# martingoe/physics

Hardware: AMD Instinct MI355X
Metric: rigid_body_steps_per_sec (higher is better)
Workload: dtype f32; 1 GPU; C5_256000_tower; n_bodies=256000, bodies_per_gpu=256000, dt_nanos=16666667, preroll_steps=30, rccl_ranks=0

## Files before the change

physics_amd/csrc/abi.hip:

```cpp
#include <algorithm>
#include <atomic>
#include <cmath>
#include <cstdlib>
#include <cstring>
#include <limits>
#include <string>
#include <vector>

#include "kernels.hpp"

namespace phys {
static thread_local std::string g_error;
void set_error(const std::string& msg) { g_error = msg; }
const char* get_error() { return g_error.c_str(); }
}

using namespace phys;

namespace phys {
void poll_snapshots(phys_world* w);
StepCounters* snapshot_acquire(phys_world* w) {
    const uint32_t k = w->snap_next;
    if (w->snap_pending[k]) {
        (void)hipEventSynchronize(w->snap_event[k]);
// ... 32 lines not shown
        hint.full_rounds = c.color_rounds;
    } else if (exact) {
        hint.color_rounds = c.color_rounds;
    } else {
        hint.recent_new[hint.recent_pos % 8] = c.n_new_manifolds;
        hint.recent_rounds[hint.recent_pos++ % 8] = c.color_rounds;
        uint32_t mx = 0, mn = 0;
        for (int q = 0; q < 8; ++q) {
            mx = hint.recent_rounds[q] > mx ? hint.recent_rounds[q] : mx;
            mn = hint.recent_new[q] > mn ? hint.recent_new[q] : mn;
        }
        hint.color_rounds = mx;
        hint.n_new = mn;
    }
    for (int q = 0; q < kMaxColors; ++q) hint.color_count[q] = c.color_count[q];
}

void poll_snapshots(phys_world* w) {
    for (int i = 0; i < phys_world::kSnapRing; ++i) {
        const uint32_t k = (w->snap_next + i) % phys_world::kSnapRing;
        if (!w->snap_pending[k]) continue;
        if (hipEventQuery(w->snap_event[k]) != hipSuccess) {
            (void)hipGetLastError();
            continue;
        }
        const StepCounters& c = *w->h_snap[k];
        w->snap_pending[k] = false;
        w->host_sticky_overflow |= c.overflow | c.sticky_overflow;
        if (c.n_static_pairs > w->static_pairs_seen) w->static_pairs_seen = c.n_static_pairs;
        if (c.overflow) continue;
        hint_adopt(w->hint, c, w->snap_full[k], false);
    }
}
}

namespace phys {
static std::atomic<int> g_worlds[64];
int worlds_on_device(int device) { return g_worlds[device & 63].load(std::memory_order_relaxed); }
bool gpu_is_exclusive(const phys_world* w) {
    return (w->cfg.flags & PHYS_FLAG_EXCLUSIVE_GPU) && !(w->cfg.flags & PHYS_FLAG_SHARED_GPU) && worlds_on_device(w->device) == 1;
}

static PlanInputs plan_inputs(const phys_world* w) {
    PlanInputs in;
    in.flags = w->cfg.flags; in.solver_iterations = w->cfg.solver_iterations;
    in.n = w->n; in.n_owned = w->n_owned; in.max_manifolds = w->max_manifolds;
    in.grid_table_size = w->grid_table_size;
    in.cus = w->cus;
    in.exclusive = gpu_is_exclusive(w);
    in.warm = w->warm;
    in.flow_vel = w->flow_vel.p != nullptr;
    in.cluster_count = w->cluster_count; in.cluster_dynamic = w->cluster_dynamic;
    in.ctab_valid = w->ctab_valid; in.color_epoch = w->color_epoch;
    uint64_t st_cap = 0;
    const uint32_t* st_pairs = nullptr;
    const float* st_geo = nullptr;
    static_narrow_args(w, &st_cap, &st_pairs, &st_geo);
    const uint64_t n_ground = (w->cfg.flags & PHYS_FLAG_GROUND_PLANE) ? (uint32_t)w->n : 0u;
    in.statics = st_pairs != nullptr;
    in.capsules = w->body_capsules || (in.statics && w->static_capsules) || w->max_ghosts > 0;
    in.filters = w->body_filters_set || (in.statics && w->static_filters_set) || (n_ground && w->ground_filter_set) || w->max_ghosts > 0;
    in.materials = materials_active(w);
    in.np_items = n_ground + w->max_pairs + st_cap;
    return in;
}

template <class Parse>
static auto debug_env(const char* name, Parse parse) -> std::optional<decltype(parse(""))> {
    if (const char* v = getenv(name)) return parse(v);
    return std::nullopt;
}
static bool debug_set(const char* name) { return getenv(name) != nullptr; }
static uint64_t parse_u64(const char* v) { return strtoull(v, nullptr, 10); }
static bool parse_one(const char* v) { return v[0] == '1'; }

const DebugSwitches& debug_switches() {
    static const DebugSwitches d = [] {
        DebugSwitches s;
        s.no_cluster = debug_set("PHYS_DEBUG_NO_CLUSTER");
        s.cluster_min = debug_env("PHYS_DEBUG_CLUSTER_MIN", parse_u64);
        s.clusters_per_cu = debug_env("PHYS_DEBUG_CLUSTERS_PER_CU", atoi);
        s.cluster_dynamic = debug_set("PHYS_DEBUG_CLUSTER_DYNAMIC");
        s.cluster_cap = debug_env("PHYS_DEBUG_CLUSTER_CAP", parse_u64).value_or(0);
        s.flow_max = debug_env("PHYS_DEBUG_FLOW_MAX", parse_u64);
        s.flow_quad_max = debug_env("PHYS_DEBUG_FLOW_QUAD_MAX", parse_u64).value_or(0);
        s.flow_pipeline = debug_env("PHYS_DEBUG_FLOW_PIPELINE", parse_one);
        s.np_early_probe = debug_env("PHYS_DEBUG_NP_EARLY_PROBE", parse_one);
        s.no_flow_preference = debug_set("PHYS_DEBUG_NO_FLOW_PREFERENCE");
        s.flow_stall = debug_set("PHYS_DEBUG_FLOW_STALL");
        s.flow_epoch = debug_env("PHYS_DEBUG_FLOW_EPOCH", [](const char* v) { return (uint32_t)strtoul(v, nullptr, 0); }).value_or(0u);
        s.ctab_slots = debug_env("PHYS_DEBUG_CTAB_SLOTS", parse_u64).value_or(0);
        s.color_kernel_lane = debug_env("PHYS_DEBUG_COLOR_KERNEL", [](const char* v) { return v[0] == 'l'; });
        s.np_threads = debug_env("PHYS_DEBUG_NP_THREADS", atoi).value_or(0);
        s.pair_lanes = debug_env("PHYS_DEBUG_PAIR_LANES", atoi).value_or(0);
        s.pair_kernel_brick = debug_env("PHYS_DEBUG_PAIR_KERNEL", [](const char* v) { return v[0] != 'b' || v[1] == 'r'; });
        s.brick_stage = debug_env("PHYS_DEBUG_BRICK_STAGE", atoi).value_or(0);
        s.raycast_stats = debug_set("PHYS_DEBUG_RAYCAST_STATS");
        return s;
    }();
    return d;
}
}

static float duration_as_secs_f32(uint64_t nanos_total) {
    const uint64_t secs = nanos_total / 1000000000ull;
    const uint32_t nanos = (uint32_t)(nanos_total % 1000000000ull);
    return (float)secs + (float)nanos / 1.0e9f;
}

phys_world::~phys_world() {
    (void)hipSetDevice(device);
    if (stream) (void)hipStreamSynchronize(stream);
    prof.destroy();
    for (int k = 0; k < kSnapRing; ++k) {
        if (h_snap[k]) (void)hipHostFree(h_snap[k]);
        if (snap_event[k]) (void)hipEventDestroy(snap_event[k]);
    }
    if (h_counters) (void)hipHostFree(h_counters);
    if (stream) (void)hipStreamDestroy(stream);
}

template <typename T>
static int32_t upload_pairs(phys_world* w, DevBuf<T>& dst, const std::vector<T>& h, bool& set_flag) {
    if (!h.empty()) PHYS_HIP_TRY(hipMemcpyAsync(dst.p, h.data(), sizeof(T) * h.size(), hipMemcpyHostToDevice, w->stream));
    PHYS_HIP_TRY(hipStreamSynchronize(w->stream));
    set_flag = true;
    return PHYS_OK;
}
template <typename T>
static int32_t download_body_pairs(phys_world* w, const DevBuf<T>& src, std::vector<T>& h) {
    h.resize(2 * w->n_owned);
    if (!h.empty()) PHYS_HIP_TRY(hipMemcpyAsync(h.data(), src.p, sizeof(T) * h.size(), hipMemcpyDeviceToHost, w->stream));
    PHYS_HIP_TRY(hipStreamSynchronize(w->stream));
    return PHYS_OK;
}

struct Staging : StageLayout {
    phys_world* w;
    DevBuf<uint8_t>& buf;
    Staging(phys_world* w, DevBuf<uint8_t>& buf) : w(w), buf(buf) {}
    int32_t reserve() {
        if (refused) return fail(PHYS_ERR_INVALID_ARG, "more arrays than a staging buffer holds");
        PHYS_HIP_TRY(buf.resize(total));
        return PHYS_OK;
    }
    template <typename T>
    T* at(Slot<T> s) const { return StageLayout::at(buf.p, s); }
    int32_t copy(hipMemcpyKind kind) {
        for (int k = 0; k < count; ++k) {
            const Array& a = arrays[k];
            if (kind == hipMemcpyHostToDevice) PHYS_HIP_TRY(hipMemcpyAsync(buf.p + a.offset, a.host, a.bytes, kind, w->stream));
            else PHYS_HIP_TRY(hipMemcpyAsync(a.host, buf.p + a.offset, a.bytes, kind, w->stream));
        }
        return PHYS_OK;
    }
};

template <class Batch, class... Kind>
static int32_t query_device(phys_world* w, const Batch& b, Kind... kind) {
    ENTER(w);
    if (const char* bad = args_error(kind..., b)) return fail(PHYS_ERR_INVALID_ARG, bad);
    if (b.n == 0) return PHYS_OK;
    return launch_query(w, kind..., b);
}

template <class Batch, class... Kind>
// ... 1073 lines not shown
```

physics_amd/csrc/cluster.hip:

```cpp
#include <algorithm>
#include <cstdio>
#include <cstdlib>
#include <mutex>
#include <vector>

#include "handoff.hpp"

namespace phys {


static size_t seg_count_offset(uint64_t n) { return ((size_t)2 * n + 3) & ~(size_t)3; }

int32_t cluster_assign(phys_world* w, const float* pos ) {
    w->cluster_count = 0;
    w->seg_count_dirty = false;
    w->seg_count_bins = 0;
    const uint64_t n = w->n, n_owned = w->n_owned;
    const DebugSwitches& dbg = debug_switches();
    w->cluster_dynamic = false;
    w->cluster_homes_valid = false;
    if (dbg.no_cluster || n_owned < kClusterMinBodies || !w->flow_vel.p) return PHYS_OK;
    const int per_cu_max = cluster_per_cu_max(w->all_diag_inertia);
    const ClusterFit fit = cluster_fit(n_owned, cluster_per_cu_first(per_cu_max, dbg), w->cus, 0u);
    if (dbg.cluster_dynamic || !fit.ok) {
// ... 106 lines not shown
                if (seen == 0xFFFFFFFFu || seen == key) break;
                s = (s + 1u) & (uint32_t)(kKeysSlots - 1);
            }
            my_slot[j] = s;
            my_rank[j] = atomicAdd(&t_cnt[s], 1u);
            if (hb != kNoHome && hb != owner) atomicOr(&body_shared[2 * (size_t)b + (c >> 5)], 1u << (c & 31u));
        }
        __syncthreads();
        for (uint32_t s = threadIdx.x; s < (uint32_t)kKeysSlots; s += 256u)
            if (t_cnt[s]) t_base[s] = atomicAdd(&seg_count[t_key[s]], t_cnt[s]);
        __syncthreads();
#pragma unroll
        for (int j = 0; j < kKeysItems; ++j) {
            const uint64_t m = base + (uint64_t)j * 256u + threadIdx.x;
            if (m < M) man_rank[m] = my_slot[j] == 0xFFFFFFFFu ? 0xFFFFFFFFu : t_base[my_slot[j]] + my_rank[j];
        }
        __syncthreads();
    }
    __syncthreads();
    if (threadIdx.x < PHYS_MAX_COLORS) {
        const uint32_t cnt = s_hist[threadIdx.x];
        if (cnt) atomicAdd(&ctr->color_count[threadIdx.x], cnt);
        const unsigned long long live = __ballot(cnt != 0u);
        if (threadIdx.x == 0 && live) atomicMax(&ctr->n_colors, 64u - (uint32_t)__clzll((long long)live));
    }
}

__global__ __launch_bounds__(256) void k_cluster_place(uint64_t max_manifolds, const uint32_t* __restrict__ man_a,
                                                       const uint32_t* __restrict__ man_b, const uint32_t* __restrict__ man_color,
                                                       const uint32_t* __restrict__ cluster_slot, uint32_t slots, uint32_t clusters,
                                                       const uint32_t* __restrict__ seg_start, const uint32_t* __restrict__ man_rank,
                                                       uint32_t* __restrict__ row_src, const StepCounters* __restrict__ ctr,
                                                       StepCounters* snap_out ) {
    counters_snapshot(ctr, snap_out);
    const uint32_t raw = ctr->n_manifolds;
    const uint32_t M = (uint64_t)raw < max_manifolds ? raw : (uint32_t)max_manifolds;
    for (uint32_t m = blockIdx.x * blockDim.x + threadIdx.x; m < M; m += gridDim.x * blockDim.x) {
        const uint32_t r = man_rank[m];
        if (r == 0xFFFFFFFFu) continue;
        const uint32_t a = man_a[m], b = man_b[m];
        const uint32_t ha = cluster_home(cluster_slot, a, slots);
        const uint32_t hb = (ha != kNoHome || PHYS_IS_STATIC_PARTNER(b)) ? kNoHome : cluster_home(cluster_slot, b, slots);
        row_src[seg_start[cluster_row_owner(a, ha, hb, clusters) * PHYS_MAX_COLORS + man_color[m]] + r] = m;
    }
}


void launch_cluster_sort(phys_world* w, const ColorPlan& plan, StepCounters* snap_out) {
    hipStream_t s = w->stream;
    const uint32_t bins = w->cluster_count * PHYS_MAX_COLORS;
    PHYS_PROF(w, PHYS_STAGE_ROWS);
    if (w->cluster_dynamic && w->cluster_homes_valid) ++w->cluster_age;
    if (w->cluster_dynamic && !w->cluster_homes_valid) {
        w->cluster_homes_valid = true;
        w->cluster_age = 0;
        const uint32_t n = (uint32_t)w->n, homes = w->cluster_count * w->cluster_slots;
        const dim3 g((n + 255) / 256), b(256);
        (void)hipMemsetAsync(w->active_flag.p, 0, ((size_t)n + 4) * 4, s);
        (void)hipMemsetAsync(w->cluster_body.p, 0xFF, (size_t)homes * 4, s);
        hipLaunchKernelGGL(k_active_flags, g, b, 0, s, (uint32_t)w->n_owned, w->color_state.p, w->bucket_of.p, w->bucket_cursor.p,
                           w->bucket_start.p, w->active_flag.p);
        const uint32_t n4 = (n + 3u) & ~3u;
        launch_exclusive_scan(w, w->active_flag.p, n4, w->active_rank.p, false, w->scan_block_sums.p);
        hipLaunchKernelGGL(k_cluster_homes, g, b, 0, s, n, (uint32_t)w->n_owned, w->color_state.p, w->bucket_of.p, w->bucket_cursor.p,
                           w->bucket_start.p, w->active_rank.p, n4, homes, w->cluster_slot.p, w->cluster_body.p, w->counters.p);
    }
    const bool self_zeroing = scan_is_one_launch(bins) && !w->seg_count_dirty;
    w->seg_count_dirty = !scan_is_one_launch(bins);
    uint32_t* seg_count = w->body_shared.p + seg_count_offset(w->n);
    (void)hipMemsetAsync(w->body_shared.p, 0, self_zeroing ? (size_t)w->n * 8 : (seg_count_offset(w->n) + (size_t)std::max<uint32_t>(bins, w->seg_count_bins)) * 4, s);
    w->seg_count_bins = bins;
    hipLaunchKernelGGL(k_cluster_keys, dim3(plan.cluster_key_blocks), dim3(256), 0, s, w->max_manifolds, w->man_a.p, w->man_b.p, w->man_color.p,
                       w->cluster_slot.p, w->cluster_slots, w->cluster_count, seg_count, w->man_rank.p, w->body_shared.p, w->counters.p);
    launch_exclusive_scan(w, seg_count, bins, w->seg_start.p, scan_is_one_launch(bins), w->scan_block_sums.p);
    hipLaunchKernelGGL(k_cluster_place, dim3(plan.cluster_sort_blocks), dim3(256), 0, s, w->max_manifolds, w->man_a.p, w->man_b.p, w->man_color.p,
                       w->cluster_slot.p, w->cluster_slots, w->cluster_count, w->seg_start.p, w->man_rank.p, w->row_src.p, w->counters.p, snap_out);
}

struct ClusterRowArrays { float4* all; uint64_t cap; };

__device__ __forceinline__ void cluster_loads_landed() { __builtin_amdgcn_s_waitcnt(0x0F70); }

constexpr int kClusterThreads = 256;
template <bool DIAG, bool GUARDED, bool MAT>
__global__ __launch_bounds__(kClusterThreads, DIAG ? kClusterPerCuDiag : kClusterPerCuFull) void k_solve_cluster(StepCounters* ctr, uint32_t iterations, uint32_t epoch,
                                                                  ClusterRowArrays rows, float friction,
                                                                  const float* __restrict__ inv_inertia, uint32_t inertia_stride,
                                                                  float* vel, const float* __restrict__ pos, float* flow_vel, uint32_t n_bodies,
                                                                  const uint32_t* __restrict__ cluster_body,
                                                                  const uint32_t* __restrict__ body_shared,
                                                                  const uint32_t* __restrict__ seg_start, uint32_t slots,
                                                                  long long timeout_ticks, uint32_t attempt,
                                                                  uint32_t last_attempt, long long arrive_ticks,
                                                                  uint32_t warm_sweep , const uint32_t* __restrict__ row_src,
                                                                  float* __restrict__ man_imp ) {
    extern __shared__ __attribute__((aligned(16))) float4 s_lds[];
    float4* s_body = s_lds;
    uint32_t* s_seg = reinterpret_cast<uint32_t*>(s_lds + 4 * (size_t)slots);
    if (ctr->overflow) return;
    if (GUARDED && attempt != 0u && ctr->cluster_state[attempt - 1u] == 1u) return;
    const uint32_t cluster = blockIdx.x;
    const uint32_t n_colors = ctr->n_colors;
    const size_t cap = (size_t)rows.cap;
    const Handoff hv = body_handoff(flow_vel, n_bodies, epoch);
    const float tag_none = __uint_as_float(hv.tag(0u));
    for (uint32_t sl = threadIdx.x; sl < slots; sl += kClusterThreads) {
        const uint32_t body = cluster_body[(size_t)cluster * slots + sl];
        float4 a = make_float4(0.0f, 0.0f, 0.0f, tag_none), b = make_float4(0.0f, 0.0f, 0.0f, 0.0f), c = b, e = b;
        if (body != 0xFFFFFFFFu) {
            const float4 v0 = reinterpret_cast<const float4*>(vel)[2 * (size_t)body];
            const float4 v1 = reinterpret_cast<const float4*>(vel)[2 * (size_t)body + 1];
            const v3 x = ld3(pos, body);
            a = make_float4(v0.x, v0.y, v0.z, tag_none);
            b = make_float4(v1.x, v1.y, v1.z, v0.w);
            c = make_float4(x.x, x.y, x.z, 0.0f);
            if (DIAG) e = reinterpret_cast<const float4*>(inv_inertia)[body * inertia_stride];
        }
        s_body[4 * sl] = a;
        s_body[4 * sl + 1] = b;
        s_body[4 * sl + 2] = c;
        s_body[4 * sl + 3] = e;
    }
    if (threadIdx.x <= (uint32_t)PHYS_MAX_COLORS) s_seg[threadIdx.x] = seg_start[(size_t)cluster * PHYS_MAX_COLORS + threadIdx.x];
    if (!GUARDED) {
        __syncthreads();
    } else {
        __shared__ uint32_t s_go;
        if (threadIdx.x == 0) {
            bool solved = false;
            for (uint32_t a = 0; a < attempt; ++a) solved = solved || __hip_atomic_load(&ctr->cluster_state[a], __ATOMIC_RELAXED, __HIP_MEMORY_SCOPE_AGENT) == 1u;
            uint32_t st = solved ? 2u : (arrive_ticks < 0 ? 1u : 0u);
            if (!solved && arrive_ticks >= 0) {
                atomicAdd(&ctr->cluster_arrived[attempt][blockIdx.x & 7u], 1u);
                const long long t0 = wall_clock64();
                for (;;) {
                    st = __hip_atomic_load(&ctr->cluster_state[attempt], __ATOMIC_RELAXED, __HIP_MEMORY_SCOPE_AGENT);
                    if (st != 0u) break;
                    uint32_t in = 0;
#pragma unroll
                    for (int k = 0; k < 8; ++k) in += __hip_atomic_load(&ctr->cluster_arrived[attempt][k], __ATOMIC_RELAXED, __HIP_MEMORY_SCOPE_AGENT);
                    if (in >= gridDim.x) {
                        atomicCAS(&ctr->cluster_state[attempt], 0u, 1u);
                    } else if (wall_clock64() - t0 > arrive_ticks) {
                        if (atomicCAS(&ctr->cluster_state[attempt], 0u, 2u) == 0u && last_attempt) flag_overflow(ctr, kOvfHandoff);
                    } else {
                        __builtin_amdgcn_s_sleep(16);
                    }
                }
            }
            s_go = st == 1u ? 1u : 0u;
        }
        __syncthreads();
        if (!s_go) return;
    }
    const long long t_start = wall_clock64();
    bool dead = false;
    const uint32_t steps = iterations * n_colors;
    const uint32_t row_base = s_seg[0], row_end = s_seg[n_colors];
    uint32_t d = row_base + threadIdx.x;
    uint32_t lit = 0;
    bool have = d < row_end && iterations != 0u;
    float4 hraw, nn, geo[4], acc[3], mas[3], fb, fi;
    auto fetch = [&]() {
        const float4* row = rows.all + d;
        hraw = row[kClusterPlaneHdr * cap];
        nn = row[kClusterPlaneN * cap];
        fb = row[kClusterPlaneForeignB * cap];
        if (DIAG) fi = row[(kClusterPlaneForeignB + 1) * cap];
#pragma unroll
        for (int k = 0; k < 4; ++k) geo[k] = row[(kClusterPlaneGeo + k) * cap];
#pragma unroll
        for (int k = 0; k < 3; ++k) {
            acc[k] = make_float4(0.0f, 0.0f, 0.0f, 0.0f);
            mas[k] = acc[k];
            if (lit != 0u || warm_sweep != 0u) acc[k] = row[(kClusterPlaneAcc + k) * cap];
            if (lit != 0u) mas[k] = row[(kClusterPlaneMass + k) * cap];
        }
    };
    hraw = make_float4(0.0f, 0.0f, 0.0f, 0.0f); nn = hraw; fb = hraw; fi = hraw;
#pragma unroll
    for (int k = 0; k < 4; ++k) geo[k] = hraw;
#pragma unroll
    for (int k = 0; k < 3; ++k) { acc[k] = hraw; mas[k] = hraw; }
    if (have) fetch();
    uint32_t it = 0, col = 0;
    for (uint32_t step = 0; step < steps; ++step) {
        const bool last_it = it + 1 == iterations;
        {
            const uint32_t seg_hi = s_seg[col + 1];
            while (have && lit == it && d < seg_hi) {
                const uint32_t d_row = d;
                const uint32_t hw = __float_as_uint(hraw.w);
                const uint4 h = MAT ? make_uint4(__float_as_uint(hraw.x), __float_as_uint(hraw.y), ticket_count(hw), ticket_without_count(hw))
                                    : make_uint4(__float_as_uint(hraw.x), __float_as_uint(hraw.y), __float_as_uint(hraw.z), hw);
                const ClusterSide sideA = cluster_side_decode(__float_as_uint(nn.w), false), sideB = cluster_side_decode(__float_as_uint(nn.w), true);
                const uint32_t modeA = sideA.mode, modeB = sideB.mode, slotA = sideA.slot, slotB = sideB.slot;
                const bool pubA = sideA.publish, pubB = sideB.publish;
                geo_manifold_t gm;
                gm.count = (int)h.z;
                gm.has_b = !PHYS_IS_STATIC_PARTNER(h.y);
                gm.n = v3_make(nn.x, nn.y, nn.z);
                tangent_basis(gm.n, &gm.t1, &gm.t2);
                impulses_unpack(acc[0], acc[1], acc[2], gm.pn, gm.pt0, gm.pt1);
                {
                    float m_t1[4], m_t2[4], m_n[4];
                    impulses_unpack(mas[0], mas[1], mas[2], m_t1, m_t2, m_n);
#pragma unroll
                    for (int k = 0; k < 4; ++k) {
                        gm.pt[k] = v3_make(geo[k].x, geo[k].y, geo[k].z);
                        gm.bias[k] = geo[k].w;
                        gm.mass[k][0] = m_t1[k]; gm.mass[k][1] = m_t2[k]; gm.mass[k][2] = m_n[k];
                    }
                }
                const RowTicket tk = ticket_decode(h.w);
                const uint32_t rankA = tk.rankA, degA = tk.degA, rankB = tk.rankB, degB = tk.degB;
                const uint32_t tA = it * degA + rankA, tB = it * degB + rankB;
                const bool finalA = last_it && rankA + 1 == degA, finalB = last_it && rankB + 1 == degB;
                v3 vA, wA, xA, vB = v3_make(0.0f, 0.0f, 0.0f), wB = vB, xB = vB;
                float ima, imb = 0.0f;
                bool needA = false, needB = false;
                m33 IA, IB;
#pragma unroll
                for (int k = 0; k < 9; ++k) { IA.m[k] = 0.0f; IB.m[k] = 0.0f; }
                v3 vA0 = v3_make(0.0f, 0.0f, 0.0f);
                vA = vA0; wA = vA0; xA = vA0; ima = 0.0f;
                if (cluster_side_at_home(modeA)) {
                    const float4* sa = s_body + 4 * slotA;
                    const float4 la = sa[0], lb = sa[1], lc = sa[2];
                    vA = v3_make(la.x, la.y, la.z); wA = v3_make(lb.x, lb.y, lb.z); ima = lb.w;
                    xA = v3_make(lc.x, lc.y, lc.z);
                    if (DIAG) { const float4 li = sa[3]; IA.m[0] = li.x; IA.m[4] = li.y; IA.m[8] = li.z; }
                    if (modeA == kSideShared) needA = __float_as_uint(la.w) != hv.tag(tA);
                } else {
                    const float4 fa = rows.all[(size_t)kClusterPlaneForeignA * cap + d_row];
                    xA = v3_make(fa.x, fa.y, fa.z); ima = fa.w;
                    if (DIAG) {
                        const float4 fia = rows.all[(size_t)(kClusterPlaneForeignA + 1) * cap + d_row];
                        IA.m[0] = fia.x; IA.m[4] = fia.y; IA.m[8] = fia.z;
                    }
                    if (tA == 0u) { const BodyVel A0 = ld_vel(vel, h.x); vA = A0.v; wA = A0.w; }
                    needA = tA != 0u;
                    cluster_loads_landed();
                }
                if (cluster_side_at_home(modeB)) {
                    const float4* sb = s_body + 4 * slotB;
                    const float4 la = sb[0], lb = sb[1], lc = sb[2];
                    vB = v3_make(la.x, la.y, la.z); wB = v3_make(lb.x, lb.y, lb.z); imb = lb.w;
                    xB = v3_make(lc.x, lc.y, lc.z);
                    if (DIAG) { const float4 li = sb[3]; IB.m[0] = li.x; IB.m[4] = li.y; IB.m[8] = li.z; }
                    if (modeB == kSideShared) needB = __float_as_uint(la.w) != hv.tag(tB);
                } else if (modeB == kSideForeign) {
                    xB = v3_make(fb.x, fb.y, fb.z); imb = fb.w;
                    if (DIAG) { IB.m[0] = fi.x; IB.m[4] = fi.y; IB.m[8] = fi.z; }
                    if (tB == 0u) {
                        const BodyVel B0 = ld_vel(vel, h.y);
                        vB = B0.v; wB = B0.w;
                        cluster_loads_landed();
                    }
                    needB = tB != 0u;
                }
                if (!DIAG) {
                    IA = ld_inertia<false>(inv_inertia, h.x * inertia_stride);
                    if (gm.has_b) IB = ld_inertia<false>(inv_inertia, h.y * inertia_stride);
                }
                uint32_t sweeps = 0, late = 0, gap;
                while (needA || needB) {
                    if (needA) needA = !take_body(hv, ld_body(hv, h.x), tA, vA, wA, gap);
                    if (needB) needB = !take_body(hv, ld_body(hv, h.y), tB, vB, wB, gap);
                    if (needA || needB) {
                        __builtin_amdgcn_s_sleep(kClusterPollSleep);
                        if ((++sweeps & 63u) == 0u && handoff_give_up(ctr, t_start, timeout_ticks)) {
                            late = (needA ? 1u : 0u) | (needB ? 2u : 0u);
                            flag_overflow(ctr, kOvfHandoff); dead = true; needA = false; needB = false;
                        }
                    }
                }
                if (GUARDED && late && atomicCAS(&ctr->debug[0], 0u, kClusterTimeoutMark) == 0u) {
                    cluster_timeout_note_encode(ClusterTimeoutNote{cluster, gridDim.x, d_row, h.x, h.y, tA, tB, late & 1u, late >> 1, modeA, modeB, col, it},
                                                ctr->debug);
                }
                cluster_loads_landed();
                if (!dead) {
                    const float fr = MAT ? hraw.z : friction;
                    if (it != 0u) solve_manifold_flat<false, false>(&gm, fr, xA, ima, &IA, xB, imb, &IB, &vA, &wA, &vB, &wB);
                    else if (warm_sweep == 0u) solve_manifold_flat<true, false>(&gm, fr, xA, ima, &IA, xB, imb, &IB, &vA, &wA, &vB, &wB);
                    else solve_manifold_flat<true, true>(&gm, fr, xA, ima, &IA, xB, imb, &IB, &vA, &wA, &vB, &wB);
                    if (cluster_side_at_home(modeA)) {
                        s_body[4 * slotA] = make_float4(vA.x, vA.y, vA.z, __uint_as_float(hv.tag(tA + 1u)));
                        s_body[4 * slotA + 1] = make_float4(wA.x, wA.y, wA.z, ima);
                    }
                    if (modeA == kSideShared || modeA == kSideForeign) {
                        if (finalA) { st3(vel + 8 * (size_t)h.x, 0, vA); st3(vel + 8 * (size_t)h.x + 4, 0, wA); }
                        else if (modeA == kSideForeign || pubA) publish_body(hv, h.x, vA, wA, tA + 1u);
                    }
                    if (cluster_side_at_home(modeB)) {
                        s_body[4 * slotB] = make_float4(vB.x, vB.y, vB.z, __uint_as_float(hv.tag(tB + 1u)));
                        s_body[4 * slotB + 1] = make_float4(wB.x, wB.y, wB.z, imb);
                    }
                    if (modeB == kSideShared || modeB == kSideForeign) {
                        if (finalB) { st3(vel + 8 * (size_t)h.y, 0, vB); st3(vel + 8 * (size_t)h.y + 4, 0, wB); }
                        else if (modeB == kSideForeign || pubB) publish_body(hv, h.y, vB, wB, tB + 1u);
                    }
                    float4 a0, a1, a2;
                    impulses_pack(gm.pn, gm.pt0, gm.pt1, a0, a1, a2);
                    if (last_it && man_imp) {
                        float4* o = reinterpret_cast<float4*>(man_imp) + kImpulseVecs * (size_t)row_src[d_row];
                        o[0] = a0; o[1] = a1; o[2] = a2;
                    }
                    if (!last_it) {
                        float4* out = rows.all + d_row;
                        out[(kClusterPlaneAcc + 0) * cap] = a0;
                        if (gm.count > 1) out[(kClusterPlaneAcc + 1) * cap] = a1;
                        if (gm.count > 2) out[(kClusterPlaneAcc + 2) * cap] = a2;
                        if (it == 0u) {
                            const float m_t1[4] = {gm.mass[0][0], gm.mass[1][0], gm.mass[2][0], gm.mass[3][0]};
                            const float m_t2[4] = {gm.mass[0][1], gm.mass[1][1], gm.mass[2][1], gm.mass[3][1]};
                            const float m_n[4] = {gm.mass[0][2], gm.mass[1][2], gm.mass[2][2], gm.mass[3][2]};
                            float4 m0, m1, m2;
                            impulses_pack(m_t1, m_t2, m_n, m0, m1, m2);
                            out[(kClusterPlaneMass + 0) * cap] = m0;
                            if (gm.count > 1) out[(kClusterPlaneMass + 1) * cap] = m1;
                            if (gm.count > 2) out[(kClusterPlaneMass + 2) * cap] = m2;
                        }
                    }
                }
                d += kClusterThreads;
                if (d >= row_end) {
                    d = row_base + threadIdx.x; ++lit;
                    if (d == d_row) asm volatile("s_waitcnt vmcnt(0)" ::: "memory");
                }
                have = lit < iterations && !dead;
                if (have) fetch();
            }
            if (seg_hi != s_seg[col]) asm volatile("s_waitcnt lgkmcnt(0)\n\ts_barrier" ::: "memory");
        }
        if (++col == n_colors) { col = 0u; ++it; }
    }
    for (uint32_t sl = threadIdx.x; sl < slots; sl += kClusterThreads) {
        const uint32_t body = cluster_body[(size_t)cluster * slots + sl];
        if (body == 0xFFFFFFFFu || (body_shared[2 * (size_t)body] | body_shared[2 * (size_t)body + 1])) continue;
        const float4 a = s_body[4 * sl], b = s_body[4 * sl + 1];
        st3(vel + 8 * (size_t)body, 0, v3_make(a.x, a.y, a.z));
        st3(vel + 8 * (size_t)body + 4, 0, v3_make(b.x, b.y, b.z));
    }
}

void launch_solve_cluster(phys_world* w, const SolverPlan& plan, void* row_all, uint64_t cap, float friction, const float* inertia,
                          uint32_t stride, bool diag) {
    const uint32_t warm_sweep = w->warm ? 1u : 0u;
    const uint32_t sweeps = w->cfg.solver_iterations + warm_sweep;
    ClusterRowArrays rows;
    rows.all = (float4*)row_all; rows.cap = cap;
    const size_t lds = cluster_lds_bytes(w->cluster_slots);
    const dim3 g(w->cluster_count), b(kClusterThreads);
    static std::mutex chain_lock;
    static hipEvent_t chain_event[64] = {};
    std::lock_guard<std::mutex> hold(chain_lock);
    {
        static bool attr_set[64] = {};
        const hipError_t e = allow_dynamic_lds(attr_set, w->device, {
            reinterpret_cast<const void*>(&k_solve_cluster<true, true, false>), reinterpret_cast<const void*>(&k_solve_cluster<true, false, false>),
            reinterpret_cast<const void*>(&k_solve_cluster<false, true, false>), reinterpret_cast<const void*>(&k_solve_cluster<false, false, false>),
            reinterpret_cast<const void*>(&k_solve_cluster<true, true, true>), reinterpret_cast<const void*>(&k_solve_cluster<true, false, true>),
            reinterpret_cast<const void*>(&k_solve_cluster<false, true, true>), reinterpret_cast<const void*>(&k_solve_cluster<false, false, true>)}, 160 * 1024);
        if (e != hipSuccess) set_error(std::string("hipFuncSetAttribute(k_solve_cluster): ") + hipGetErrorString(e));
    }
    hipEvent_t& ev = chain_event[w->device & 63];
    if (ev) (void)hipStreamWaitEvent(w->stream, ev, 0);
    else (void)hipEventCreateWithFlags(&ev, hipEventDisableTiming);
    struct Record { hipEvent_t e; hipStream_t s; ~Record() { if (e) (void)hipEventRecord(e, s); } } record{ev, w->stream};
    dispatch_bool(diag, [&](auto diag_t) { dispatch_bool(plan.guarded, [&](auto guarded_t) { dispatch_bool(plan.materials, [&](auto mat_t) {
        constexpr bool D = decltype(diag_t)::value, G = decltype(guarded_t)::value, MT = decltype(mat_t)::value;
        const uint32_t kAttempts = G ? 2u : 1u;
        for (uint32_t attempt = 0; attempt < kAttempts; ++attempt) {
            const uint32_t last = attempt + 1 == kAttempts ? 1u : 0u;
            const long long arrive_ticks = !G ? -1ll : (attempt == 0 ? 50000ll : 2000000ll);
            hipLaunchKernelGGL((k_solve_cluster<D, G, MT>), g, b, lds, w->stream, w->counters.p, sweeps, w->flow_epoch, rows, friction,
                               inertia, stride, w->vel.p, w->pos.p, w->flow_vel.p, (uint32_t)w->n, w->cluster_body.p,
                               w->body_shared.p, w->seg_start.p, w->cluster_slots, plan.timeout_ticks, attempt, last, arrive_ticks,
                               warm_sweep, w->row_src.p, w->warm ? w->man_imp.p : (float*)nullptr);
        }
    }); }); });
}

}
```

physics_amd/csrc/plan.hpp:

```cpp
#pragma once
#include <algorithm>
#include <cstddef>
#include <cstdint>
#include <optional>

#include "../../include/physics_hip.h"

namespace phys {

constexpr int kMaxColors = 64;
constexpr int kColorCachePeriod = 64;
constexpr uint32_t kHandoffIterationsEnd = 1000;

struct StepHint {
    bool valid = false;
    uint32_t n_manifolds = 0, n_colors = 0, n_pairs = 0, max_region = 0, n_used_buckets = 0, n_contacts = 0;
    uint32_t n_active = 0;
    uint32_t color_rounds = 0;
    uint32_t full_rounds = 0;
    uint32_t recent_rounds[8] = {};
    uint32_t recent_pos = 0;
    uint32_t n_new = 0xFFFFFFFFu;
    uint32_t recent_new[8] = {};
    uint32_t color_count[kMaxColors] = {};
};

struct DebugSwitches {
    bool no_cluster = false, cluster_dynamic = false, no_flow_preference = false, flow_stall = false;
    std::optional<uint64_t> cluster_min, flow_max;
    std::optional<int> clusters_per_cu;
    uint64_t cluster_cap = 0, flow_quad_max = 0, ctab_slots = 0;
    uint32_t flow_epoch = 0;
    int np_threads = 0, pair_lanes = 0, brick_stage = 0;
    bool raycast_stats = false;
    std::optional<bool> flow_pipeline, np_early_probe;
    std::optional<bool> color_kernel_lane;
    std::optional<bool> pair_kernel_brick;
};

struct PlanInputs {
    uint32_t flags = 0, solver_iterations = 0;
    uint64_t n = 0, n_owned = 0, max_manifolds = 0;
    uint32_t grid_table_size = 0;
    int cus = 0;
    bool exclusive = false;
    bool warm = false;
    bool flow_vel = false;
    uint32_t cluster_count = 0;
    bool cluster_dynamic = false;
    bool ctab_valid = false;
    uint64_t color_epoch = 0;
    bool statics = false, capsules = false, filters = false, materials = false;
    uint64_t np_items = 0;
};

constexpr int kPairThreads = 256;
constexpr int kRegX = 6, kRegY = 6, kRegZ = 5, kRegCells = kRegX * kRegY * kRegZ;
constexpr int kColorThreads = 1024;
constexpr int kSmallTrips = 40;
constexpr int kSortBlocksMax = 512;
constexpr int kSortChunk = 4096;
constexpr int kKeysItems = 4;
constexpr int kQuadRowsPerGroup = 64;
constexpr int kEventThreads = 256;

constexpr uint32_t kSlotGridMaxBodies = 32768;
constexpr uint64_t kClusterMinBodies = 32768;
constexpr uint64_t kClusterMinManifolds = 170000;
constexpr long long kFlowTimeoutTicks = 300000000ll;
constexpr uint64_t kFlowMaxManifolds = 400000;
constexpr uint64_t kFlowQuadMaxManifolds = 200000;
constexpr uint32_t kTailMax = 512;
constexpr uint32_t kQuadColorMaxRows = 32768;
constexpr uint32_t kBrickCapMax = 5000;
constexpr size_t kBrickPerCuMax = 7;

inline bool flow_quad_beats_cluster(uint32_t manifolds, uint32_t contacts, uint32_t colors) {
    if (!colors || !contacts) return false;
    const double flow = 8.4e-8 * manifolds + 1.86e-8 * contacts + 0.0009 * colors;
    const double cluster = 1.1 * std::max(0.0041 * colors, 6.9e-8 * manifolds);
    return flow < cluster;
}

enum class PairKernel { Slots, Brick128, Brick256, Lanes4, Lanes1 };
struct PairPlan {
    PairKernel kernel = PairKernel::Slots;
    uint32_t cap = 0;
    size_t lds = 0;
    uint32_t wgs = 0;
};
inline PairPlan plan_pairs(const PlanInputs& in, const StepHint& h, const DebugSwitches& dbg) {
    PairPlan p;
    const uint32_t n = (uint32_t)in.n;
    const uint32_t per_four_lanes = (uint32_t)(((uint64_t)n * 4 + kPairThreads - 1) / kPairThreads);
    if (n <= kSlotGridMaxBodies) {
        p.kernel = PairKernel::Slots;
        p.wgs = per_four_lanes;
        return p;
    }
    const bool crowded = h.valid && h.n_used_buckets && (uint64_t)in.n * 10ull > (uint64_t)h.n_used_buckets * 21ull;
    const bool brick = dbg.pair_kernel_brick.value_or(!crowded);
    if (brick && !dbg.pair_lanes) {
        const uint32_t n_bricks = in.grid_table_size >> 6;
        uint32_t cap = h.valid && h.max_region ? h.max_region + h.max_region / 4 : 1024u;
        cap = std::min(std::max((cap + 63u) & ~63u, 256u), kBrickCapMax);
        const size_t dyn = (size_t)cap * 28;
        const bool small_stage = dbg.brick_stage ? dbg.brick_stage == 128 : (h.valid && (uint64_t)h.n_pairs < 3ull * in.n);
        const size_t fixed = (kPairThreads / 64) * (small_stage ? 128 : 256) * 8 + kRegCells * 8 + 64;
        const uint32_t per_cu = (uint32_t)std::min<size_t>(kBrickPerCuMax, (160 * 1024) / (((dyn + fixed) + 1023) / 1024 * 1024));
        uint32_t wgs = 256u * std::max(per_cu, 1u);
        while (wgs > n_bricks) wgs >>= 1;
        p.kernel = small_stage ? PairKernel::Brick128 : PairKernel::Brick256;
        p.cap = cap;
        p.lds = dyn;
        p.wgs = wgs;
        return p;
    }
    if (dbg.pair_lanes ? dbg.pair_lanes == 4 : n <= 65536u) {
        p.kernel = PairKernel::Lanes4;
        p.wgs = per_four_lanes;
// ... 151 lines not shown
```

physics_amd/csrc/setup.hpp:

```cpp
#pragma once
#include <algorithm>
#include <cmath>
#include <cstddef>
#include <cstdint>
#include <cstring>
#include <limits>
#include <optional>
#include <string>
#include <utility>
#include <vector>

#include "../../include/physics_hip.h"
#include "../../include/spec/collide.h"
#include "../../include/spec/contact_solve.h"
#include "../../include/spec/det_math.h"
#include "../../include/spec/body_edit.h"
#include "../../include/spec/force_field.h"
#include "../../include/spec/liquid.h"
#include "../../include/spec/vec.h"
#include "plan.hpp"

namespace phys {

struct StepCounters {
// ... 47 lines not shown
    float target[3];
};

struct GridShape {
    uint32_t mx = 7, my = 7, mz = 7;
    uint32_t sx = 1, sy = 1;
};
struct GridPlan {
    uint32_t table_size = 0;
    GridShape shape;
};
inline uint32_t table_bits_for(uint64_t n) {
    uint32_t bits = 9;
    while ((1ull << bits) < 2 * n && bits < 27) ++bits;
    return bits;
}
inline GridPlan grid_plan(uint64_t n_total, uint64_t n_owned, const float* pos, const float* half_extent, float contact_margin) {
    const uint64_t n = n_owned;
    const uint32_t bits = table_bits_for(n_total);
    GridPlan out;
    out.table_size = 1u << bits;
    float lo[3] = {3e38f, 3e38f, 3e38f}, hi[3] = {-3e38f, -3e38f, -3e38f}, diam = 0.0f;
    for (uint64_t i = 0; i < n; ++i) {
        for (int a = 0; a < 3; ++a) { lo[a] = std::min(lo[a], pos[3 * i + a]); hi[a] = std::max(hi[a], pos[3 * i + a]); }
        if (half_extent) {
            const float* h = half_extent + 3 * i;
            diam = std::max(diam, 2.0f * std::max(h[0], std::max(h[1], h[2])));
        }
    }
    const float cell = (diam > 0.0f ? diam : 1.0f) * 1.05f + 2.0f * contact_margin;
    double cells[3];
    for (int a = 0; a < 3; ++a) cells[a] = n ? std::max(1.0, (double)(hi[a] - lo[a]) / cell + 1.0) : 1.0;
    uint32_t ab[3] = {2, 2, 2};
    for (uint32_t left = bits - 6; left > 0; --left) {
        int best = 0;
        double worst = -1.0;
        for (int a = 0; a < 3; ++a) {
            const double load = cells[a] / (double)(1u << ab[a]);
            if (load > worst && ab[a] < 20) { worst = load; best = a; }
        }
        ab[best] += 1;
    }
    GridShape& g = out.shape;
    g.mx = (1u << ab[0]) - 1u; g.my = (1u << ab[1]) - 1u; g.mz = (1u << ab[2]) - 1u;
    g.sx = ab[0] - 2u; g.sy = ab[1] - 2u;
    return out;
}

struct CollisionSizes {
    uint64_t max_pairs = 0, max_manifolds = 0;
    bool ok = false;
    uint64_t ctab_slots = 0;
    bool warm = false;
    bool flow_buffers = false;
    size_t bucket_bytes = 0, color_bytes = 0, counter_bytes = sizeof(StepCounters);
};
inline CollisionSizes collision_sizes(const phys_config& cfg, uint64_t n_total, const DebugSwitches& dbg) {
    CollisionSizes s;
    const uint64_t n = n_total;
    s.max_pairs = cfg.max_pairs ? cfg.max_pairs : std::max<uint64_t>(24 * n, 4096);
    s.max_manifolds = cfg.max_manifolds ? cfg.max_manifolds : std::max<uint64_t>(17 * n, 4096);
    s.ok = !(s.max_pairs > 0xFFFFFFF0ull || s.max_manifolds > 0xFFFFFFF0ull);
    const size_t T = (size_t)1 << table_bits_for(n);
    const bool contacts = !(cfg.flags & PHYS_FLAG_BROADPHASE_ONLY);
    s.bucket_bytes = (T * 4 + 255) / 256 * 256;
    s.color_bytes = contacts ? ((size_t)4 * n * 8 + 255) / 256 * 256 : 0;
    if (!contacts) return s;
    const uint64_t M = s.max_manifolds;
    s.warm = !(cfg.flags & PHYS_FLAG_NO_WARM_START) && M < (1ull << 26);
    uint64_t cap = 4096;
    while (cap < M + M / 2) cap <<= 1;
    if (dbg.ctab_slots >= 64 && (dbg.ctab_slots & (dbg.ctab_slots - 1)) == 0) cap = dbg.ctab_slots;
    s.ctab_slots = cap;
    s.flow_buffers = !(cfg.flags & PHYS_FLAG_SOLVER_PER_COLOR) && 64 * M < 0xFFFFFFFFull && 32 * n < 0xFFFFFFFFull;
    return s;
}

constexpr uint32_t kClusterDynamicPeriod = 8;
constexpr uint32_t kClusterMaxSlots = 2496;
constexpr int kClusterPerCuDiag = 3, kClusterPerCuFull = 2;
constexpr size_t kClusterLdsPerCu = 160 * 1024;
constexpr uint32_t kClusterSlotBytes = 64;
inline size_t cluster_lds_bytes(uint32_t slots) { return (size_t)slots * kClusterSlotBytes + (PHYS_MAX_COLORS + 1) * 4 + 12; }
inline uint32_t clusters_on_chip(int per_cu, int cus) { return (uint32_t)std::max(8, per_cu * (cus - cus / 8)); }
inline int cluster_per_cu_max(bool all_diag_inertia) { return all_diag_inertia ? kClusterPerCuDiag : kClusterPerCuFull; }
inline int cluster_per_cu_first(int per_cu_max, const DebugSwitches& dbg) {
    return dbg.clusters_per_cu ? std::min(per_cu_max, std::max(1, *dbg.clusters_per_cu)) : per_cu_max;
}

struct ClusterFit {
    int per_cu = 0;
    uint32_t clusters = 0, slots = 0;
    bool ok = false;
};
inline ClusterFit cluster_fit(uint64_t want_bodies, int per_cu_first, int cus, uint32_t min_slots) {
    ClusterFit f;
    for (f.per_cu = per_cu_first;; --f.per_cu) {
        f.clusters = clusters_on_chip(f.per_cu, cus);
        f.slots = (uint32_t)((want_bodies + f.clusters - 1) / f.clusters);
        f.slots = std::max(min_slots, (f.slots + 63u) / 64u * 64u);
        const size_t per_wg = (cluster_lds_bytes(f.slots) + 1023) / 1024 * 1024;
        f.ok = per_wg * (size_t)f.per_cu <= kClusterLdsPerCu && f.slots <= kClusterMaxSlots;
        if (f.ok || f.per_cu <= 1) return f;
    }
}

struct ClusterHomes {
    uint32_t clusters = 0;
    std::vector<uint32_t> cluster_slot;
    std::vector<uint32_t> cluster_body;
};
inline uint32_t spread10(uint32_t x) {
    x &= 0x3ffu;
    x = (x ^ (x << 16)) & 0xff0000ffu;
    x = (x ^ (x << 8)) & 0x0300f00fu;
    x = (x ^ (x << 4)) & 0x030c30c3u;
    x = (x ^ (x << 2)) & 0x09249249u;
    return x;
}
inline ClusterHomes cluster_homes(uint64_t n_total, uint64_t n_owned, const float* pos, uint32_t slots) {
    ClusterHomes out;
    out.clusters = (uint32_t)((n_owned + slots - 1) / slots);
    float lo[3] = {3e38f, 3e38f, 3e38f}, hi[3] = {-3e38f, -3e38f, -3e38f};
    for (uint64_t i = 0; i < n_owned; ++i)
        for (int a = 0; a < 3; ++a) { lo[a] = std::min(lo[a], pos[3 * i + a]); hi[a] = std::max(hi[a], pos[3 * i + a]); }
    const float span = std::max(std::max(hi[0] - lo[0], hi[1] - lo[1]), std::max(hi[2] - lo[2], 1e-6f));
    const float scale = 1023.0f / span;
    std::vector<uint64_t> keyed(n_owned);
    for (uint64_t i = 0; i < n_owned; ++i) {
        uint32_t q[3];
        for (int a = 0; a < 3; ++a) {
            const float t = (pos[3 * i + a] - lo[a]) * scale;
            q[a] = t <= 0.0f ? 0u : (t >= 1023.0f ? 1023u : (uint32_t)t);
        }
        const uint64_t key = spread10(q[0]) | (spread10(q[1]) << 1) | (spread10(q[2]) << 2);
        keyed[i] = (key << 32) | i;
    }
    std::sort(keyed.begin(), keyed.end());
    out.cluster_slot.assign(n_total, 0xFFFFFFFFu);
    out.cluster_body.assign((size_t)out.clusters * slots, 0xFFFFFFFFu);
    for (uint64_t r = 0; r < n_owned; ++r) {
        const uint32_t i = (uint32_t)keyed[r];
        out.cluster_slot[i] = (uint32_t)r;
        out.cluster_body[r] = i;
    }
    return out;
}

struct ClusterShape { uint32_t clusters = 0, slots = 0; };
inline std::optional<ClusterShape> plan_dynamic_clusters(uint64_t n_owned, bool all_diag_inertia, int cus, const StepHint& h,
                                                         const DebugSwitches& dbg) {
    uint64_t active = h.n_active;
    if (active == 0) active = std::min<uint64_t>(n_owned, (uint64_t)h.n_manifolds);
    if (active == 0) return std::nullopt;
    const int per_cu_max = cluster_per_cu_max(all_diag_inertia);
    uint64_t want = active + active / 4;
    if (dbg.cluster_cap && want > dbg.cluster_cap) want = dbg.cluster_cap;
    const ClusterFit f = cluster_fit(want, cluster_per_cu_first(per_cu_max, dbg), cus, 64u);
    if ((!f.ok || f.per_cu < per_cu_max) && !dbg.cluster_cap && !dbg.clusters_per_cu) return std::nullopt;
    if (!f.ok && !dbg.cluster_cap) return std::nullopt;
    ClusterShape s;
    s.clusters = f.clusters;
    s.slots = f.ok ? f.slots : kClusterMaxSlots / 64u * 64u;
    return s;
}

constexpr uint32_t kStMaxDim = 1024;
constexpr uint32_t kStLargeCells = 64;

PHYS_HD uint32_t st_cell(float x, float org, float inv, uint32_t dim) {
    float t = floorf((x - org) * inv);
    if (!(t >= 0.0f)) t = 0.0f;
    const float top = (float)(dim - 1u);
    t = t > top ? top : t;
    return (uint32_t)t;
}

struct StaticSet {
    std::vector<float> geo;
    std::vector<float> rc;
    std::vector<float> box;
    std::vector<uint32_t> cell_start, cell_ids;
    std::vector<uint32_t> large;
    uint32_t n_large = 0;
    float org[3] = {0.0f, 0.0f, 0.0f}, inv_cell = 0.0f;
    uint32_t dim[3] = {0, 0, 0};
    bool capsules = false;
// ... 500 lines not shown
```

Baseline: 239.6 million body-steps/s.

## Deal cluster solver rows to waves in per-color 64-row blocks

```diff
diff --git a/physics_amd/csrc/abi.hip b/physics_amd/csrc/abi.hip
--- a/physics_amd/csrc/abi.hip
+++ b/physics_amd/csrc/abi.hip
@@ -138,6 +138,7 @@
         s.clusters_per_cu = debug_env("PHYS_DEBUG_CLUSTERS_PER_CU", atoi);
         s.cluster_dynamic = debug_set("PHYS_DEBUG_CLUSTER_DYNAMIC");
         s.cluster_cap = debug_env("PHYS_DEBUG_CLUSTER_CAP", parse_u64).value_or(0);
+        s.cluster_deal_rows = debug_env("PHYS_DEBUG_CLUSTER_DEAL", [](const char* v) { return v[0] == 'r'; }).value_or(false);
         s.flow_max = debug_env("PHYS_DEBUG_FLOW_MAX", parse_u64);
         s.flow_quad_max = debug_env("PHYS_DEBUG_FLOW_QUAD_MAX", parse_u64).value_or(0);
         s.flow_pipeline = debug_env("PHYS_DEBUG_FLOW_PIPELINE", parse_one);
diff --git a/physics_amd/csrc/cluster.hip b/physics_amd/csrc/cluster.hip
--- a/physics_amd/csrc/cluster.hip
+++ b/physics_amd/csrc/cluster.hip
@@ -212,7 +212,9 @@
 __device__ __forceinline__ void cluster_loads_landed() { __builtin_amdgcn_s_waitcnt(0x0F70); }
 
 constexpr int kClusterThreads = 256;
-template <bool DIAG, bool GUARDED, bool MAT>
+static_assert((uint32_t)kClusterThreads == kClusterLanes && kClusterBlock == 64u && PHYS_MAX_COLORS == 64,
+              "the dealing of setup.hpp is this kernel's: 256 lanes, blocks of one wave, a segment table one wave scans");
+template <bool DIAG, bool GUARDED, bool MAT, bool BLOCKS>
 __global__ __launch_bounds__(kClusterThreads, DIAG ? kClusterPerCuDiag : kClusterPerCuFull) void k_solve_cluster(StepCounters* ctr, uint32_t iterations, uint32_t epoch,
                                                                   ClusterRowArrays rows, float friction,
                                                                   const float* __restrict__ inv_inertia, uint32_t inertia_stride,
@@ -227,6 +229,7 @@
     extern __shared__ __attribute__((aligned(16))) float4 s_lds[];
     float4* s_body = s_lds;
     uint32_t* s_seg = reinterpret_cast<uint32_t*>(s_lds + 4 * (size_t)slots);
+    __shared__ uint32_t s_vseg[BLOCKS ? PHYS_MAX_COLORS + 1 : 1];
     if (ctr->overflow) return;
     if (GUARDED && attempt != 0u && ctr->cluster_state[attempt - 1u] == 1u) return;
     const uint32_t cluster = blockIdx.x;
@@ -252,6 +255,11 @@
         s_body[4 * sl + 3] = e;
     }
     if (threadIdx.x <= (uint32_t)PHYS_MAX_COLORS) s_seg[threadIdx.x] = seg_start[(size_t)cluster * PHYS_MAX_COLORS + threadIdx.x];
+    if (BLOCKS && threadIdx.x < (uint32_t)PHYS_MAX_COLORS) {
+        const uint32_t* seg = seg_start + (size_t)cluster * PHYS_MAX_COLORS + threadIdx.x;
+        s_vseg[threadIdx.x + 1u] = wave_inclusive_scan(cluster_block_span(seg[1] - seg[0]));
+        if (threadIdx.x == 0u) s_vseg[0] = 0u;
+    }
     if (!GUARDED) {
         __syncthreads();
     } else {
@@ -287,8 +295,13 @@
     bool dead = false;
     const uint32_t steps = iterations * n_colors;
     const uint32_t row_base = s_seg[0], row_end = s_seg[n_colors];
+    const uint32_t lane = threadIdx.x & 63u;
+    const auto wave_v0 = [] { return (uint32_t)__builtin_amdgcn_readfirstlane((int)(threadIdx.x & ~63u)); };
+    const uint32_t vend = BLOCKS ? (uint32_t)__builtin_amdgcn_readfirstlane((int)s_vseg[n_colors]) : 0u;
+    uint32_t vb = BLOCKS ? wave_v0() : 0u, cs = 0;
     uint32_t d = row_base + threadIdx.x;
     uint32_t lit = 0;
+    uint32_t d_row = kClusterNoRow;
     bool have = d < row_end && iterations != 0u;
     float4 hraw, nn, geo[4], acc[3], mas[3], fb, fi;
     auto fetch = [&]() {
@@ -312,14 +325,42 @@
     for (int k = 0; k < 4; ++k) geo[k] = hraw;
 #pragma unroll
     for (int k = 0; k < 3; ++k) { acc[k] = hraw; mas[k] = hraw; }
-    if (have) fetch();
+    const auto vseg_at = [&](uint32_t c) { return (uint32_t)__builtin_amdgcn_readfirstlane((int)s_vseg[c]); };
+    auto block_enter = [&](bool advance) {
+        have = false;
+        bool wrapped = false;
+        if (advance) {
+            vb += kClusterThreads;
+            wrapped = vb >= vend;
+            if (wrapped) { vb = wave_v0(); cs = 0u; ++lit; }
+        }
+        if (lit >= iterations) return;
+        while (vseg_at(cs + 1u) <= vb) ++cs;
+        const uint32_t lo = (uint32_t)__builtin_amdgcn_readfirstlane((int)s_seg[cs]), hi = (uint32_t)__builtin_amdgcn_readfirstlane((int)s_seg[cs + 1u]);
+        const uint32_t vlo = vseg_at(cs);
+        d = cluster_block_row(lo, hi, vlo, vb + lane);
+        have = d != kClusterNoRow && !dead;
+        if (have) {
+            if (wrapped && d == d_row) asm volatile("s_waitcnt vmcnt(0)" ::: "memory");
+            fetch();
+        } else {
+            hraw.x = 0.0f; hraw.y = 0.0f;
+            nn.w = __uint_as_float(cluster_sides_encode(cluster_side_encode(0u, 0u, kSideOwn), cluster_side_encode(0u, 0u, kSideNone)));
+        }
+    };
+    if (BLOCKS) {
+        if (vb >= vend) lit = iterations;
+        block_enter(false);
+    } else if (have) {
+        fetch();
+    }
     uint32_t it = 0, col = 0;
     for (uint32_t step = 0; step < steps; ++step) {
         const bool last_it = it + 1 == iterations;
         {
             const uint32_t seg_hi = s_seg[col + 1];
-            while (have && lit == it && d < seg_hi) {
-                const uint32_t d_row = d;
+            while (BLOCKS ? (lit == it && cs == col) : (have && lit == it && d < seg_hi)) {
+                d_row = d;
                 const uint32_t hw = __float_as_uint(hraw.w);
                 const uint4 h = MAT ? make_uint4(__float_as_uint(hraw.x), __float_as_uint(hraw.y), ticket_count(hw), ticket_without_count(hw))
                                     : make_uint4(__float_as_uint(hraw.x), __float_as_uint(hraw.y), __float_as_uint(hraw.z), hw);
@@ -410,7 +451,7 @@
                                                 ctr->debug);
                 }
                 cluster_loads_landed();
-                if (!dead) {
+                if (!dead && (!BLOCKS || have)) {
                     const float fr = MAT ? hraw.z : friction;
                     if (it != 0u) solve_manifold_flat<false, false>(&gm, fr, xA, ima, &IA, xB, imb, &IB, &vA, &wA, &vB, &wB);
                     else if (warm_sweep == 0u) solve_manifold_flat<true, false>(&gm, fr, xA, ima, &IA, xB, imb, &IB, &vA, &wA, &vB, &wB);
@@ -454,6 +495,10 @@
                         }
                     }
                 }
+                if (BLOCKS) {
+                    block_enter(true);
+                    continue;
+                }
                 d += kClusterThreads;
                 if (d >= row_end) {
                     d = row_base + threadIdx.x; ++lit;
@@ -462,7 +507,7 @@
                 have = lit < iterations && !dead;
                 if (have) fetch();
             }
-            if (seg_hi != s_seg[col]) asm volatile("s_waitcnt lgkmcnt(0)\n\ts_barrier" ::: "memory");
+            if ((BLOCKS ? s_seg[col + 1] : seg_hi) != s_seg[col]) asm volatile("s_waitcnt lgkmcnt(0)\n\ts_barrier" ::: "memory");
         }
         if (++col == n_colors) { col = 0u; ++it; }
     }
@@ -488,29 +533,32 @@
     std::lock_guard<std::mutex> hold(chain_lock);
     {
         static bool attr_set[64] = {};
-        const hipError_t e = allow_dynamic_lds(attr_set, w->device, {
-            reinterpret_cast<const void*>(&k_solve_cluster<true, true, false>), reinterpret_cast<const void*>(&k_solve_cluster<true, false, false>),
-            reinterpret_cast<const void*>(&k_solve_cluster<false, true, false>), reinterpret_cast<const void*>(&k_solve_cluster<false, false, false>),
-            reinterpret_cast<const void*>(&k_solve_cluster<true, true, true>), reinterpret_cast<const void*>(&k_solve_cluster<true, false, true>),
-            reinterpret_cast<const void*>(&k_solve_cluster<false, true, true>), reinterpret_cast<const void*>(&k_solve_cluster<false, false, true>)}, 160 * 1024);
+#define PHYS_CLUSTER_INSTANCES(BLOCKS)                                                                                                                     \
+    reinterpret_cast<const void*>(&k_solve_cluster<true, true, false, BLOCKS>), reinterpret_cast<const void*>(&k_solve_cluster<true, false, false, BLOCKS>),   \
+    reinterpret_cast<const void*>(&k_solve_cluster<false, true, false, BLOCKS>), reinterpret_cast<const void*>(&k_solve_cluster<false, false, false, BLOCKS>), \
+    reinterpret_cast<const void*>(&k_solve_cluster<true, true, true, BLOCKS>), reinterpret_cast<const void*>(&k_solve_cluster<true, false, true, BLOCKS>),     \
+    reinterpret_cast<const void*>(&k_solve_cluster<false, true, true, BLOCKS>), reinterpret_cast<const void*>(&k_solve_cluster<false, false, true, BLOCKS>)
+        const hipError_t e = allow_dynamic_lds(attr_set, w->device, {PHYS_CLUSTER_INSTANCES(true), PHYS_CLUSTER_INSTANCES(false)}, 160 * 1024);
+#undef PHYS_CLUSTER_INSTANCES
         if (e != hipSuccess) set_error(std::string("hipFuncSetAttribute(k_solve_cluster): ") + hipGetErrorString(e));
     }
     hipEvent_t& ev = chain_event[w->device & 63];
     if (ev) (void)hipStreamWaitEvent(w->stream, ev, 0);
     else (void)hipEventCreateWithFlags(&ev, hipEventDisableTiming);
     struct Record { hipEvent_t e; hipStream_t s; ~Record() { if (e) (void)hipEventRecord(e, s); } } record{ev, w->stream};
-    dispatch_bool(diag, [&](auto diag_t) { dispatch_bool(plan.guarded, [&](auto guarded_t) { dispatch_bool(plan.materials, [&](auto mat_t) {
-        constexpr bool D = decltype(diag_t)::value, G = decltype(guarded_t)::value, MT = decltype(mat_t)::value;
+    const bool blocks = !debug_switches().cluster_deal_rows;
+    dispatch_bool(diag, [&](auto diag_t) { dispatch_bool(plan.guarded, [&](auto guarded_t) { dispatch_bool(plan.materials, [&](auto mat_t) { dispatch_bool(blocks, [&](auto blocks_t) {
+        constexpr bool D = decltype(diag_t)::value, G = decltype(guarded_t)::value, MT = decltype(mat_t)::value, BL = decltype(blocks_t)::value;
         const uint32_t kAttempts = G ? 2u : 1u;
         for (uint32_t attempt = 0; attempt < kAttempts; ++attempt) {
             const uint32_t last = attempt + 1 == kAttempts ? 1u : 0u;
             const long long arrive_ticks = !G ? -1ll : (attempt == 0 ? 50000ll : 2000000ll);
-            hipLaunchKernelGGL((k_solve_cluster<D, G, MT>), g, b, lds, w->stream, w->counters.p, sweeps, w->flow_epoch, rows, friction,
+            hipLaunchKernelGGL((k_solve_cluster<D, G, MT, BL>), g, b, lds, w->stream, w->counters.p, sweeps, w->flow_epoch, rows, friction,
                                inertia, stride, w->vel.p, w->pos.p, w->flow_vel.p, (uint32_t)w->n, w->cluster_body.p,
                                w->body_shared.p, w->seg_start.p, w->cluster_slots, plan.timeout_ticks, attempt, last, arrive_ticks,
                                warm_sweep, w->row_src.p, w->warm ? w->man_imp.p : (float*)nullptr);
         }
-    }); }); });
-}
-
-}
+    }); }); }); });
+}
+
+}
diff --git a/physics_amd/csrc/plan.hpp b/physics_amd/csrc/plan.hpp
--- a/physics_amd/csrc/plan.hpp
+++ b/physics_amd/csrc/plan.hpp
@@ -36,6 +36,7 @@
     std::optional<bool> flow_pipeline, np_early_probe;
     std::optional<bool> color_kernel_lane;
     std::optional<bool> pair_kernel_brick;
+    bool cluster_deal_rows = false;
 };
 
 struct PlanInputs {
diff --git a/physics_amd/csrc/setup.hpp b/physics_amd/csrc/setup.hpp
--- a/physics_amd/csrc/setup.hpp
+++ b/physics_amd/csrc/setup.hpp
@@ -153,6 +153,8 @@
 constexpr size_t kClusterLdsPerCu = 160 * 1024;
 constexpr uint32_t kClusterSlotBytes = 64;
 inline size_t cluster_lds_bytes(uint32_t slots) { return (size_t)slots * kClusterSlotBytes + (PHYS_MAX_COLORS + 1) * 4 + 12; }
+constexpr size_t kClusterLdsStatic = (PHYS_MAX_COLORS + 1) * 4 + 16;
+inline size_t cluster_lds_footprint(uint32_t slots) { return cluster_lds_bytes(slots) + kClusterLdsStatic; }
 inline uint32_t clusters_on_chip(int per_cu, int cus) { return (uint32_t)std::max(8, per_cu * (cus - cus / 8)); }
 inline int cluster_per_cu_max(bool all_diag_inertia) { return all_diag_inertia ? kClusterPerCuDiag : kClusterPerCuFull; }
 inline int cluster_per_cu_first(int per_cu_max, const DebugSwitches& dbg) {
@@ -170,10 +172,42 @@
         f.clusters = clusters_on_chip(f.per_cu, cus);
         f.slots = (uint32_t)((want_bodies + f.clusters - 1) / f.clusters);
         f.slots = std::max(min_slots, (f.slots + 63u) / 64u * 64u);
-        const size_t per_wg = (cluster_lds_bytes(f.slots) + 1023) / 1024 * 1024;
+        const size_t per_wg = (cluster_lds_footprint(f.slots) + 1023) / 1024 * 1024;
         f.ok = per_wg * (size_t)f.per_cu <= kClusterLdsPerCu && f.slots <= kClusterMaxSlots;
         if (f.ok || f.per_cu <= 1) return f;
     }
+}
+
+#ifdef __HIPCC__
+#define PHYS_SETUP_HD __host__ __device__ __forceinline__
+#else
+#define PHYS_SETUP_HD inline
+#endif
+constexpr uint32_t kClusterLanes = 256, kClusterBlock = 64, kClusterNoRow = 0xFFFFFFFFu;
+PHYS_SETUP_HD uint32_t cluster_block_span(uint32_t rows) { return (rows + (kClusterBlock - 1u)) & ~(kClusterBlock - 1u); }
+PHYS_SETUP_HD uint32_t cluster_block_row(uint32_t lo, uint32_t hi, uint32_t vlo, uint32_t v) {
+    const uint32_t d = lo + (v - vlo);
+    return d < hi ? d : kClusterNoRow;
+}
+inline void cluster_block_starts(const uint32_t* seg, uint32_t* vseg) {
+    vseg[0] = 0u;
+    for (int c = 0; c < PHYS_MAX_COLORS; ++c) vseg[c + 1] = vseg[c] + cluster_block_span(seg[c + 1] - seg[c]);
+}
+struct ClusterDeal { uint64_t rows = 0, blocks = 0; };
+inline ClusterDeal cluster_deal_count(const uint32_t* seg, uint32_t n_colors) {
+    ClusterDeal out;
+    const auto owned_below = [](uint32_t l, uint32_t x) { return x > l ? (x - l + kClusterLanes - 1u) / kClusterLanes : 0u; };
+    for (uint32_t c = 0; c < n_colors && c < (uint32_t)PHYS_MAX_COLORS; ++c) {
+        const uint32_t lo = seg[c] - seg[0], hi = seg[c + 1] - seg[0];
+        for (uint32_t wave = 0; wave < kClusterLanes / kClusterBlock; ++wave) {
+            uint32_t busiest = 0;
+            for (uint32_t l = wave * kClusterBlock; l < (wave + 1u) * kClusterBlock; ++l)
+                busiest = std::max(busiest, owned_below(l, hi) - owned_below(l, lo));
+            out.rows += busiest;
+        }
+        out.blocks += cluster_block_span(hi - lo) / kClusterBlock;
+    }
+    return out;
 }
 
 struct ClusterHomes {
```

Measured after the change: 237.4 million body-steps/s. No clear change (-0.9%).
